# mightypirate1/DRL-Tetris

Hardware: AMD Instinct MI355X
Metric: env-steps/sec at 64k parallel 20x10 boards (higher is better)
Workload: dtype u32

## Files before the change

drl-tetris_amd/csrc/tetris_engine.h:

```cpp
#pragma once
#include "tetris_layout.h"
#include "tetris_tables.h"

#if defined(__clang__)
#define TE_UNROLL _Pragma("unroll")
#else
#define TE_UNROLL _Pragma("GCC unroll 8")
#endif

namespace te {

TE_HD int ctz32(uint32_t v) { return __builtin_ctz(v); }
TE_HD int clz32(uint32_t v) { return __builtin_clz(v); }
#if defined(__HIP_DEVICE_COMPILE__)
TE_HD uint32_t ld_stream(const uint32_t* p) { return __builtin_nontemporal_load(p); }
TE_HD void st_stream(uint32_t* p, uint32_t v) { __builtin_nontemporal_store(v, p); }
#else
TE_HD uint32_t ld_stream(const uint32_t* p) { return *p; }
TE_HD void st_stream(uint32_t* p, uint32_t v) { *p = v; }
#endif

#if defined(TE_PATH_COUNTERS) && !defined(__HIPCC__)
enum PathCounter { PC_KICK = 0, PC_KICK_2ND, PC_KICK_3RD, PC_KICK_FAILED, PC_KICK_DOWN, PC_DROP_EXACT, PC_RT_OFF_SPAWN,
                   PC_GARBAGE_ROW, PC_GARBAGE_LIFT2, PC_DEATH_GARBAGE, PC_DEATH_SPAWN, PC_TIMER_LOCK, PC_KEY_KICK, PC_KEY_KICK_FAILED,
// ... 38 lines not shown
    if (mem != MEM_STREAM) st_agent(p, v); else st_stream(p, v);
}
#endif
TE_HD uint32_t ldw(const uint32_t* base, uint32_t o, size_t word_off, int mem = MEM_STREAM) { return ldw_b(base, o, word_off * 4u, mem); }
TE_HD void stw(uint32_t* base, uint32_t o, size_t word_off, uint32_t v, int mem = MEM_STREAM) { stw_b(base, o, word_off * 4u, v, mem); }
struct RowStride { size_t ws; };
template <int N>
struct RowTable { uint32_t bytes[N]; };
TE_HD size_t row_bytes(const RowStride& r, int w) { return (size_t)w * r.ws * 4u; }
template <int N>
TE_HD size_t row_bytes(const RowTable<N>& r, int w) { return r.bytes[w]; }
#if defined(__HIP_DEVICE_COMPILE__)
TE_HD void add_word(uint32_t* p, uint32_t v) { (void)__hip_atomic_fetch_add(p, v, __ATOMIC_RELAXED, __HIP_MEMORY_SCOPE_AGENT); }
#else
TE_HD void add_word(uint32_t* p, uint32_t v) { *p += v; }
#endif
#if defined(__HIP_DEVICE_COMPILE__)
TE_HD uint32_t mul24(uint32_t a, uint32_t b) { return __umul24(a, b); }
#else
TE_HD uint32_t mul24(uint32_t a, uint32_t b) { return a * b; }
#endif
TE_HD int imin(int a, int b) { return a < b ? a : b; }
TE_HD int imax(int a, int b) { return a > b ? a : b; }
TE_HD uint32_t f2u(float f) { union { float f; uint32_t u; } v; v.f = f; return v.u; }
TE_HD float u2f(uint32_t u) { union { float f; uint32_t u; } v; v.u = u; return v.f; }

constexpr uint16_t SHAPE_ROWS[7][4] = {
    {0x2260, 0x0710, 0x3220, 0x4700}, {0x2230, 0x1700, 0x6220, 0x0740}, {0x2640, 0x0630, 0x1320, 0x6300},
    {0x2310, 0x3600, 0x4620, 0x0360}, {0x2222, 0x0f00, 0x4444, 0x00f0}, {0x0720, 0x2320, 0x2700, 0x2620},
    {0x0660, 0x0660, 0x0660, 0x0660},
};
TE_HD int spawn_rot(int kind) { return (int)((0x0977u >> (2 * (kind & 7))) & 3u); }
TE_HD int shape_value(int kind) { return (int)((0x06127534u >> (4 * (kind & 7))) & 15u); }

constexpr uint32_t make_shape(int kind, int rot) {
    uint32_t rows = SHAPE_ROWS[kind][rot];
    uint32_t nibs = 0;
    for (int gy = 0; gy < 4; gy++) {
        uint32_t rown = (rows >> (4 * (3 - gy))) & 0xF;
        for (int gx = 0; gx < 4; gx++)
            if ((rown >> gx) & 1) nibs |= 1u << (4 * gx + gy);
    }
    int minc = 3, maxc = 0;
    for (int gx = 0; gx < 4; gx++)
        if ((nibs >> (4 * gx)) & 0xF) { if (gx < minc) minc = gx; if (gx > maxc) maxc = gx; }
    return nibs | ((uint32_t)minc << 16) | ((uint32_t)maxc << 18);
}
constexpr uint32_t make_drop_word(uint32_t nibs) {
    uint32_t w = 0;
    for (int gx = 0; gx < 4; gx++) {
        uint32_t n = (nibs >> (4 * gx)) & 0xF;
        int bottom = -1;
        for (int gy = 0; gy < 4; gy++)
            if ((n >> gy) & 1) bottom = gy;
        w |= (uint32_t)(bottom < 0 ? 0x7F : 0x40 - (bottom + 1)) << (8 * gx);
    }
    return w;
}
constexpr int SHAPE_WORDS = 64;
struct ShapeTable { uint32_t s[SHAPE_WORDS]; };
constexpr ShapeTable make_shape_table() {
    ShapeTable t{};
    for (int k = 0; k < 7; k++)
        for (int r = 0; r < 4; r++) {
            t.s[k * 4 + r] = make_shape(k, r);
            t.s[32 + k * 4 + r] = make_drop_word(t.s[k * 4 + r] & 0xFFFFu);
        }
    for (int r = 0; r < 4; r++) { t.s[28 + r] = 0; t.s[60 + r] = 0x7F7F7F7Fu; }
    return t;
}
constexpr ShapeTable SHAPES = make_shape_table();

struct Ctx {
    const uint32_t* shapes;
    const uint8_t* table;
    const uint64_t* start;
    const double* combo_pow;
    uint32_t n_draws;
    uint32_t margin;
    int H;
    uint32_t floor_bits;
    bool tint;
    bool queue;
};

constexpr int ERR_FIFO = 1;
constexpr int ERR_STREAM = 2;

struct Raw8 { uint32_t lo, hi; };
struct Player {
    uint32_t col[NCOL];
    uint32_t tint[3][NCOL];
    int kind, rot, x, y, next;
    int dead, lock_armed, reward;
    int inc_count, combo_count, line_count, qlen;
    int q_overflow;
    int32_t time_ms, drop_delay, drop_time, speedup_time, lock_time;
    int32_t combo_start, combo_time, min_remaining;
    uint32_t combo_remaining;
    float incoming;
    uint32_t piece_draws, hole_draws;
    uint32_t pgroup;
    uint32_t lines_sent, lines_cleared, lines_blocked, max_combo, lines_seen, garbage_cleared;
    int32_t qcount[FIFO_CAP];
    int32_t qdelay[FIFO_CAP];
    int q_loaded;
    Raw8 pf_raw;
    int pf_ok;
};

struct ResetPrefetch { uint32_t seed16; uint64_t word; int ok; };

template <int P>
struct Game {
    Player pl[P];
    uint32_t seed16;
    int round_over, last_winner;
    uint32_t flags;
    uint32_t episode;
    uint32_t steps;
    uint32_t add_lines, add_sent;
    uint32_t status;
    uint32_t draw0, draw1;
};

template <class ROWS>
TE_HD void load_player_rows(const uint32_t* s, uint32_t o, const ROWS& rows, Player& q, bool tint, bool queue = true, int mem = MEM_STREAM) {
    for (int c = 0; c < NCOL; c++) q.col[c] = ldw_b(s, o, row_bytes(rows, W_COL0 + c), mem);
    if (tint)
        for (int k = 0; k < 3; k++)
            for (int c = 0; c < NCOL; c++) q.tint[k][c] = ldw_b(s, o, row_bytes(rows, W_TINT0 + 10 * k + c), mem);
    uint32_t w = ldw_b(s, o, row_bytes(rows, W_PIECE), mem);
    q.kind = w & 7; q.rot = (w >> 3) & 3; q.x = (int)((w >> 5) & 15) - 4; q.y = (w >> 9) & 31;
    q.next = (w >> 14) & 7; q.dead = (w >> 17) & 1; q.lock_armed = (w >> 18) & 1; q.reward = (w >> 19) & 255;
    w = ldw_b(s, o, row_bytes(rows, W_MISC), mem);
    q.inc_count = w & 255; q.combo_count = (w >> 8) & 255; q.line_count = (w >> 16) & 255;
    q.qlen = (w >> 24) & 15; q.q_overflow = (w >> 28) & 3;
    if (!queue) { q.inc_count = 0; q.qlen = 0; q.q_overflow = 0; }
    q.time_ms = (int32_t)ldw_b(s, o, row_bytes(rows, W_TIME), mem);
    w = ldw_b(s, o, row_bytes(rows, W_DROPCOMBO), mem);
    q.drop_delay = w & 0xFFFF; q.combo_remaining = w >> 16;
    q.drop_time = (int32_t)ldw_b(s, o, row_bytes(rows, W_DROP_TIME), mem);
    q.speedup_time = (int32_t)ldw_b(s, o, row_bytes(rows, W_SPEEDUP_TIME), mem);
    q.lock_time = (int32_t)ldw_b(s, o, row_bytes(rows, W_LOCK_TIME), mem);
    q.combo_start = (int32_t)ldw_b(s, o, row_bytes(rows, W_COMBO_START), mem);
    q.combo_time = (int32_t)ldw_b(s, o, row_bytes(rows, W_COMBO_TIME), mem);
    q.incoming = queue ? u2f(ldw_b(s, o, row_bytes(rows, W_INCOMING), mem)) : 0.0f;
    q.min_remaining = queue ? (int32_t)ldw_b(s, o, row_bytes(rows, W_MIN_REMAINING), mem) : 1000;
    q.piece_draws = ldw_b(s, o, row_bytes(rows, W_PIECE_DRAWS), mem);
    q.hole_draws = queue ? ldw_b(s, o, row_bytes(rows, W_HOLE_DRAWS), mem) : 0u;
    q.pgroup = ldw_b(s, o, row_bytes(rows, W_PIECE_GROUP), mem);
    w = ldw_b(s, o, row_bytes(rows, W_STATS0), mem); q.lines_sent = w & 0xFFFF; q.lines_cleared = w >> 16;
    w = ldw_b(s, o, row_bytes(rows, W_STATS1), mem); q.lines_blocked = w & 0xFFFF; q.max_combo = w >> 16;
    w = ldw_b(s, o, row_bytes(rows, W_STATS2), mem); q.lines_seen = w & 0xFFFF; q.garbage_cleared = w >> 16;
    q.q_loaded = queue && q.qlen > 0;
    q.pf_ok = 0; q.pf_raw.lo = 0; q.pf_raw.hi = 0;
    if (queue)
        for (int i = 0; i < FIFO_CAP; i++) { q.qcount[i] = 0; q.qdelay[i] = 0; }
    if (q.q_loaded) {
        for (int i = 0; i < FIFO_CAP / 2; i++) {
            uint32_t cw = ldw_b(s, o, row_bytes(rows, W_FIFO_COUNT0 + i), mem);
            q.qcount[2 * i] = (int16_t)(cw & 0xFFFF);
            q.qcount[2 * i + 1] = (int16_t)(cw >> 16);
        }
        for (int i = 0; i < FIFO_CAP; i++) q.qdelay[i] = (int32_t)ldw_b(s, o, row_bytes(rows, W_FIFO_DELAY0 + i), mem);
    }
// ... 282 lines not shown
    while (amount && q.qlen) {
        int take = imin(amount, (int)q.qcount[0]);
        if (take < 1) take = 1;
        q.qcount[0] -= take; amount -= take; blocked += take;
        if (q.qcount[0] == 0) q_pop_front(q);
    }
    q.lines_blocked = (q.lines_blocked + (uint32_t)blocked) & 0xFFFFu;
    if (q.qlen) {
        if (head_delay > q.qdelay[0]) q.qdelay[0] = head_delay;
        if (freeze) q.qdelay[0] = imin(q.qdelay[0] + 450, t + q.min_remaining + 450);
    } else
        q.min_remaining = 1000;
    return amount;
}

TE_HD bool q_release(Player& q, int32_t t) {
    if (q.qlen == 0) return false;
    if (t > q.qdelay[0]) {
        int32_t next_delay = q.qdelay[0] + 450;
        if (--q.qcount[0] == 0) q_pop_front(q);
        if (q.qlen) {
            if (next_delay > q.qdelay[0]) q.qdelay[0] = next_delay;
            q.min_remaining = q.qdelay[0] - t;
        } else
            q.min_remaining = 1000;
        return true;
    }
    q.min_remaining = imin(q.min_remaining, q.qdelay[0] - t);
    return false;
}

TE_HD int q_total(const Player& q) {
    uint32_t total = 0;
    for (int i = 0; i < FIFO_CAP; i++)
        if (i < q.qlen) total += (uint32_t)q.qcount[i];
    return (int)(total & 0xFFFFu);
}


TE_HD void combo_gain(Player& q, int32_t t, int amount) {
    if (q.combo_count == 0) { q.combo_start = t; q.combo_time = 0; }
    q.combo_count = (q.combo_count + 1) & 255;
    float line_time = 0.0f;
    for (int i = 0; i < amount; i++) {
        q.line_count = (q.line_count + 1) & 255;
        line_time = line_time + (float)(1000 / imax(1, q.line_count));
    }
    float add = (float)(800 / imax(1, q.combo_count)) + line_time;
    q.combo_time = (int32_t)((float)q.combo_time + add);
    if ((uint32_t)q.combo_count > q.max_combo) q.max_combo = (uint32_t)q.combo_count;
}

TE_HD int combo_expire(const Ctx& cx, Player& q, int32_t t) {
    int32_t left = q.combo_start + q.combo_time - t;
    q.combo_remaining = left < 0 ? 0u : ((uint32_t)left & 0xFFFFu);
    if (t > q.combo_start + q.combo_time && q.combo_count != 0) {
        float duration = 1.f + (float)t / 60000.f * 0.1f;
        double v = cx.combo_pow[q.combo_count] * (double)duration;
        int lines = (int)((uint32_t)(int64_t)v & 0xFFFFu);
        q.combo_count = 0;
        q.line_count = 0;
        return lines;
    }
    return 0;
}


TE_HD bool spawn_next(const Ctx& cx, Player& q, uint32_t seed16, uint32_t& status) {
    q.kind = q.next;
    q.rot = spawn_rot(q.kind);
    q.x = (NCOL - 4) / 2;
    q.y = 0;
    if (q.piece_draws + cx.margin >= cx.n_draws) {
        status |= ST_NEED_EXTEND;
        if (q.piece_draws >= cx.n_draws) status |= ST_STREAM_EXHAUSTED;
    }
    q.next = (int)((q.pgroup >> (4u * (q.piece_draws & 7u))) & 7u);
    q.piece_draws++;
    if ((q.piece_draws & 7u) == 0u) {
        q.pgroup = pack_group(q.pf_ok ? q.pf_raw : table_group_raw(cx, seed16, q.piece_draws, status));
        q.pf_ok = 0;
    }
    uint32_t shape = shape_of(cx, q.kind, q.rot);
    if (!fits_spawn_col(cx, q, shape, 0)) { stamp(cx, q, shape); TE_COUNT(PC_DEATH_SPAWN); return true; }
    return false;
}

TE_HD int score_clears(const Ctx& cx, Player& q, int cleared) {
    q.lines_cleared = (q.lines_cleared + (uint32_t)cleared) & 0xFFFFu;
    if (cleared == 0) { q.combo_time -= 200; return 0; }
    int amount = cx.queue ? q_block(q, cleared - 1, q.time_ms, true) : cleared - 1;
    q.lines_sent = (q.lines_sent + (uint32_t)amount) & 0xFFFFu;
    combo_gain(q, q.time_ms, cleared);
    return amount;
}

TE_HD void lock_piece(const Ctx& cx, Player& q) {
    uint32_t shape = shape_of(cx, q.kind, q.rot);
    q.y += drop_distance(cx, q, shape);
    stamp(cx, q, shape);
    q.drop_time = q.time_ms;
    q.lock_armed = 0;
}

TE_HD int settle(const Ctx& cx, Player& q, uint32_t seed16, uint32_t& status) {
    int sent = score_clears(cx, q, clear_rows(cx, q));
    if (spawn_next(cx, q, seed16, status)) return -1;
    return sent;
}

TE_HD bool soft_drop(const Ctx& cx, Player& q) {
    const uint32_t shape = shape_of(cx, q.kind, q.rot);
    if (q.x == (NCOL - 4) / 2 ? fits_spawn_col(cx, q, shape, q.y + 1) : fits_at(cx, q, shape, q.x, q.y + 1)) {
        q.y++;
        q.drop_time = q.time_ms;
        q.lock_armed = 0;
        return true;
    }
    if (!q.lock_armed) q.lock_time = q.time_ms + 400;
    q.lock_armed = 1;
    return false;
}

TE_HD bool gravity_due(Player& q, int32_t t) {
    if (t - q.speedup_time > 3000) {
        if (q.drop_delay > 200) q.drop_delay -= 10;
        else if (q.drop_delay > 100) q.drop_delay -= 5;
        else if (q.drop_delay > 50) q.drop_delay -= 2;
        else if (q.drop_delay > 10) q.drop_delay -= 1;
        q.speedup_time = t;
    }
    if (t - q.drop_time > q.drop_delay) { q.drop_time = t; return true; }
    return false;
}

TE_HD bool push_garbage(const Ctx& cx, Player& q, uint32_t seed16, uint32_t& status) {
    int hole = (int)(table_byte(cx, seed16, q.hole_draws, status) >> 4);
    q.hole_draws++;
    uint32_t bottom = 1u << (cx.H - 1);
    for (int c = 0; c < NCOL; c++) q.col[c] = (q.col[c] >> 1) | (c == hole ? 0u : bottom);
    if (cx.tint)
        for (int k = 0; k < 3; k++)
            for (int c = 0; c < NCOL; c++) q.tint[k][c] = (q.tint[k][c] >> 1) | (c == hole ? 0u : bottom);
    TE_COUNT(PC_GARBAGE_ROW);
    if (q.y > 0) q.y--;
    if (!fits_at(cx, q, shape_of(cx, q.kind, q.rot), q.x, q.y)) {
        if (q.y > 0) { q.y--; TE_COUNT(PC_GARBAGE_LIFT2); }
        else { TE_COUNT(PC_DEATH_GARBAGE); return true; }
    }
    return false;
}

TE_HD int tick(const Ctx& cx, Player& q, int ms, uint32_t seed16, uint32_t& status) {
    q.time_ms += ms;
    if (gravity_due(q, q.time_ms)) soft_drop(cx, q);
    int sent = 0;
    bool finished = false;
    if (q.lock_armed && q.time_ms > q.lock_time && !soft_drop(cx, q)) {
        TE_COUNT(PC_TIMER_LOCK);
        lock_piece(cx, q);
        sent = settle(cx, q, seed16, status);
        finished = true;
    }
    if (!finished) {
        if (cx.queue) {
            int whole = 0;
            while (q.incoming >= 1.0f) { whole++; q.incoming = q.incoming - 1.f; }
// ... 129 lines not shown
    out.r[0] = v.x; out.r[1] = v.y; out.r[2] = v.z; out.r[3] = v.w;
#else
    for (int i = 0; i < 4; i++) out.r[i] = cx.shapes[((kind & 7) << 2) | i];
#endif
    return out;
}
TE_HD Shapes4 drop_words_of_kind(const Ctx& cx, int kind) {
    Shapes4 out;
#if defined(__HIP_DEVICE_COMPILE__)
    const uint4 v = *reinterpret_cast<const uint4*>(cx.shapes + 32 + ((kind & 7) << 2));
    out.r[0] = v.x; out.r[1] = v.y; out.r[2] = v.z; out.r[3] = v.w;
#else
    for (int i = 0; i < 4; i++) out.r[i] = cx.shapes[32 + (((kind & 7) << 2) | i)];
#endif
    return out;
}
TE_HD uint32_t pick4(const Shapes4& s, int rot) {
    uint32_t lo = (rot & 1) ? s.r[1] : s.r[0];
    uint32_t hi = (rot & 1) ? s.r[3] : s.r[2];
    return (rot & 2) ? hi : lo;
}

TE_HD uint32_t free_positions32(uint64_t band, uint32_t shape) {
    const uint32_t lo = (uint32_t)band, hi = (uint32_t)(band >> 32), mid = (lo >> 16) | (hi << 16);
    const uint32_t s0 = shape & 0xFFFFu, s1 = s0 << 4, s2 = s0 << 8, s3 = s0 << 12, s4 = s0 << 16;
    uint32_t free = 0;
    free |= (s0 & lo) == 0 ? 1u << 0 : 0u;
    free |= (s1 & lo) == 0 ? 1u << 1 : 0u;
    free |= (s2 & lo) == 0 ? 1u << 2 : 0u;
    free |= (s3 & lo) == 0 ? 1u << 3 : 0u;
    free |= (s4 & lo) == 0 ? 1u << 4 : 0u;
    free |= (s1 & mid) == 0 ? 1u << 5 : 0u;
    free |= (s2 & mid) == 0 ? 1u << 6 : 0u;
    free |= (s3 & mid) == 0 ? 1u << 7 : 0u;
    free |= (s4 & mid) == 0 ? 1u << 8 : 0u;
    free |= (s1 & hi) == 0 ? 1u << 9 : 0u;
    free |= (s2 & hi) == 0 ? 1u << 10 : 0u;
    free |= (s3 & hi) == 0 ? 1u << 11 : 0u;
    free |= (s4 & hi) == 0 ? 1u << 12 : 0u;
    return free;
}
TE_HD uint32_t free_positions(uint64_t band, uint32_t shape) {
    const uint64_t pc = (uint64_t)(shape & 0xFFFFu);
    uint32_t free = 0;
    for (int xs = 0; xs <= 12; xs++) free |= (((pc << (4 * xs)) & band) == 0 ? 1u : 0u) << xs;
    return free;
}

TE_HD uint32_t band_win32(uint64_t band, int p) {
    const int off = 4 * p + 32;
    const uint32_t lo = (uint32_t)band, hi = (uint32_t)(band >> 32);
    const int k = off >> 5;
    const uint32_t a = k == 0 ? ~0u : (k == 1 ? lo : (k == 2 ? hi : ~0u));
    const uint32_t b = k == 0 ? lo : (k == 1 ? hi : ~0u);
#if defined(__HIP_DEVICE_COMPILE__)
    return __builtin_amdgcn_alignbit(b, a, (uint32_t)off & 31u);
#else
    const int sh = off & 31;
    return sh ? (a >> sh) | (b << (32 - sh)) : a;
#endif
}

struct RowsFrom { uint32_t v[NCOL]; };
TE_HD RowsFrom rows_from(const Ctx& cx, const Player& q, int y) {
    RowsFrom r;
    for (int c = 0; c < NCOL; c++) r.v[c] = (uint32_t)((int32_t)(q.col[c] | cx.floor_bits) >> y);
    return r;
}
TE_HD uint64_t band_of_rows(const RowsFrom& r) {
    uint32_t lo = 0xFFu, hi = 0xFFFF0000u;
    for (int c = 0; c < 6; c++) lo |= (r.v[c] & 0xFu) << (4 * c + 8);
    for (int c = 6; c < NCOL; c++) hi |= (r.v[c] & 0xFu) << (4 * (c - 6));
    return ((uint64_t)hi << 32) | lo;
}
TE_HD uint64_t band_one_down(uint64_t band, const RowsFrom& r) {
    uint32_t lo = (uint32_t)band, hi = (uint32_t)(band >> 32);
    lo = ((lo >> 1) & 0x77777777u) | 0xFFu;
    hi = ((hi >> 1) & 0x77777777u) | 0xFFFF0000u;
    for (int c = 0; c < 6; c++) lo |= (r.v[c] & 0x10u) << (4 * c + 7);
    hi |= (r.v[6] & 0x10u) >> 1;
    for (int c = 7; c < NCOL; c++) hi |= (r.v[c] & 0x10u) << (4 * (c - 6) - 1);
    return ((uint64_t)hi << 32) | lo;
}
TE_HD int drop_distance_rows(const Ctx& cx, const Player& q, const RowsFrom& r, uint32_t shape, uint32_t drop_word) {
    uint32_t d[NCOL];
    for (int c = 0; c < NCOL; c++) d[c] = (uint32_t)ctz32(r.v[c]);
    const uint32_t w0 = (d[0] << 16) | (d[1] << 24);
    const uint32_t w1 = d[2] | (d[3] << 8) | (d[4] << 16) | (d[5] << 24);
    const uint32_t w2 = d[6] | (d[7] << 8) | (d[8] << 16) | (d[9] << 24);
    const unsigned xs = (unsigned)(q.x + 2);
    const bool hi2 = (xs & 8u) != 0, hi1 = (xs & 4u) != 0;
    const uint32_t lo = hi2 ? (hi1 ? 0u : w2) : (hi1 ? w1 : w0);
    const uint32_t hi = hi2 ? 0u : (hi1 ? w2 : w1);
#if defined(__HIP_DEVICE_COMPILE__)
    const uint32_t under = __builtin_amdgcn_alignbyte(hi, lo, xs & 3u);
#else
    const uint32_t under = (uint32_t)((((uint64_t)hi << 32) | lo) >> (8 * (xs & 3u)));
#endif
    const uint32_t sum = under + drop_word;
    const uint32_t b0 = sum & 0xFFu, b1 = (sum >> 8) & 0xFFu, b2 = (sum >> 16) & 0xFFu, b3 = sum >> 24;
    const uint32_t m01 = b0 < b1 ? b0 : b1, m23 = b2 < b3 ? b2 : b3;
    const uint32_t m = m01 < m23 ? m01 : m23;
    if (m - 0x40u > 0x3Eu) { TE_COUNT(PC_DROP_EXACT); return drop_distance(cx, q, shape); }
    return (int)(m - 0x40u);
}

TE_HD void play_rt(const Ctx& cx, Player& q, int r, int t) {
    const Shapes4 sh = shapes_of_kind(cx, q.kind);
    const Shapes4 dw = drop_words_of_kind(cx, q.kind);
    if (q.y != 0 || q.x != (NCOL - 4) / 2) TE_COUNT(PC_RT_OFF_SPAWN);
    RowsFrom rows = rows_from(cx, q, q.y);
    uint64_t band = band_of_rows(rows);
    uint32_t win = band_win32(band, q.x);
    const bool fit1 = (((pick4(sh, q.rot + 1) & 0xFFFFu) << 8) & win) == 0;
    const bool fit2 = (((pick4(sh, q.rot + 2) & 0xFFFFu) << 8) & win) == 0;
    const bool fit3 = (((pick4(sh, q.rot + 3) & 0xFFFFu) << 8) & win) == 0;
    const bool easy = (r < 1 || fit1) && (r < 2 || fit2) && (r < 3 || fit3);
    if (easy) {
        q.rot = (q.rot + r) & 3;
    } else {
        int adv = fit1 ? (fit2 ? (fit3 ? 3 : 2) : 1) : 0;
        q.rot = (q.rot + adv) & 3;
        int left = r - adv;
        int kicks = 0;
        (void)kicks;
        while (left > 0) {
            const int nr = (q.rot + 1) & 3;
            const uint32_t s1 = pick4(sh, nr) & 0xFFFFu;
            const uint64_t b1 = band_one_down(band, rows);
            const uint32_t win1 = band_win32(b1, q.x);
            const uint32_t sA = s1, sB = s1 << 4, sC = s1 << 8, sD = s1 << 12, sE = s1 << 16;
            const bool k0 = (sC & win1) == 0, k1 = (sB & win) == 0, k2 = (sD & win) == 0;
            const bool k3 = (sB & win1) == 0, k4 = (sD & win1) == 0;
            const bool k5 = (sA & win) == 0, k6 = (sE & win) == 0;
            int dx = k6 ? 2 : 99, dy = 0;
            dx = k5 ? -2 : dx;
            if (k4) { dx = 1; dy = 1; }
            if (k3) { dx = -1; dy = 1; }
            if (k2) { dx = 1; dy = 0; }
            if (k1) { dx = -1; dy = 0; }
            if (k0) { dx = 0; dy = 1; }
            if (dx == 99) { TE_COUNT(PC_KICK_FAILED); break; }
            kicks++;
            TE_COUNT(kicks == 1 ? PC_KICK : (kicks == 2 ? PC_KICK_2ND : PC_KICK_3RD));
            if (dy) TE_COUNT(PC_KICK_DOWN);
            q.rot = nr; q.x += dx; q.y += dy;
            if (dy) {
                band = b1;
                for (int c = 0; c < NCOL; c++) rows.v[c] >>= 1;
            }
            left--;
            if (left > 0) {
                win = band_win32(band, q.x);
                const bool g1 = (((pick4(sh, q.rot + 1) & 0xFFFFu) << 8) & win) == 0;
                const bool g2 = left > 1 && (((pick4(sh, q.rot + 2) & 0xFFFFu) << 8) & win) == 0;
                const int more = g1 ? (g2 ? 2 : 1) : 0;
                q.rot = (q.rot + more) & 3;
                left -= more;
            }
        }
    }
    const uint32_t shape = pick4(sh, q.rot);
    const uint32_t free = free_positions32(band, shape);
    const int xs0 = q.x + 2;
    const uint32_t blocked_left = ~free & ((1u << xs0) - 1u);
    int xs = blocked_left ? 32 - clz32(blocked_left) : 0;
    const uint32_t blocked_right = (~free >> (xs + 1)) | (1u << 13);
    xs += imin(t, ctz32(blocked_right));
    q.x = xs - 2;
    q.y += drop_distance_rows(cx, q, rows, shape, pick4(dw, q.rot));
    stamp(cx, q, shape);
    q.drop_time = q.time_ms;
    q.lock_armed = 0;
}

constexpr int PROBE_PATH = 96;
struct Probe {
    Player q;
    int spawn;
    uint8_t path[PROBE_PATH]; int path_len;
    uint8_t best[PROBE_PATH]; int best_len, best_x, best_rot;
    uint8_t* keys; uint8_t* lens;
    int max_lists, max_keys, n_lists, overflow;
};
struct Pose { int rot, x, y; };
TE_HD Pose pose_get(const Probe& t) { Pose p = {t.q.rot, t.q.x, t.q.y}; return p; }
TE_HD void pose_set(Probe& t, Pose p) { t.q.rot = p.rot; t.q.x = p.x; t.q.y = p.y; }

TE_HD bool fits_any(const Ctx& cx, const Player& q, uint32_t shape, int x, int y) {
    if (y >= 0) return fits_at(cx, q, shape, x, y);
    int k = -y;
    if (k > 3) return (shape & 0xFFFFu) == 0;
    uint32_t low = ((1u << k) - 1u) * 0x1111u;
    if (shape & low) return false;
    return fits_at(cx, q, ((shape & 0xFFFFu) >> k) & ((0xFu >> k) * 0x1111u), x, 0);
}
TE_HD bool probe_fits(const Ctx& cx, const Probe& t) { return fits_any(cx, t.q, shape_of(cx, t.q.kind, t.q.rot), t.q.x, t.q.y); }
TE_HD bool probe_shift(const Ctx& cx, Probe& t, int dx) {
    if (fits_any(cx, t.q, shape_of(cx, t.q.kind, t.q.rot), t.q.x + dx, t.q.y)) { t.q.x += dx; return true; }
    return false;
}
TE_HD void probe_drop(const Ctx& cx, Probe& t) { t.q.y += drop_distance(cx, t.q, shape_of(cx, t.q.kind, t.q.rot)); }
TE_HD void path_push(Probe& t, int v) { if (t.path_len < PROBE_PATH) t.path[t.path_len++] = (uint8_t)v; else t.overflow = 1; }

TE_HD int convert_code(int m) {
    return m == 255 ? 3 : m == 254 ? 1 : m == 253 ? 6 : m == 252 ? 5 : m == 241 ? 8 : m == 242 ? 10 : m == 243 ? 9 : m;
}
TE_HD void emit_key(Probe& t, int& n, int code) {
    if (t.n_lists < t.max_lists && n < t.max_keys) t.keys[t.n_lists * t.max_keys + n] = (uint8_t)convert_code(code);
    else t.overflow = 1;
    n++;
}
TE_HD void emit_end(Probe& t, int n) {
    if (t.n_lists < t.max_lists) t.lens[t.n_lists] = (uint8_t)imin(n, t.max_keys);
    t.n_lists++;
}
TE_HD void emit_rotation(Probe& t, int& n, int value) { value &= 3; if (value) emit_key(t, n, 240 + value); }
TE_HD void emit_start_moves(Probe& t, int& n, int x) {
    const int mid = (NCOL - 4) / 2;
    for (int i = 0; i < x - mid; i++) emit_key(t, n, 255);
    for (int i = 0; i < mid - x; i++) emit_key(t, n, 254);
}

TE_HD int probe_move_up(const Ctx& cx, Probe& t) {
    t.q.y++;
    const bool landed = !probe_fits(cx, t);
    t.q.y--;
    int count = 0;
    do { t.q.y--; count++; } while (probe_fits(cx, t));
    count--;
    t.q.y++;
    if (count && landed) return 253;
    return count & 255;
}

TE_HD bool probe_commit(Probe& t) {
    for (int i = 0; i < t.path_len; i++) t.best[i] = t.path[i];
    t.best_len = t.path_len; t.best_x = t.q.x; t.best_rot = t.q.rot;
    return true;
// ... 276 lines not shown
```

drl-tetris_amd/csrc/tetris_kernels.h:

```cpp
#pragma once
#include "../../include/tetris_hip.h"
#include "tetris_engine.h"

namespace te {

struct KArgs {
    uint32_t* state;
    uint32_t* gstate;
    uint32_t* status;
    const uint8_t* table;
    const uint64_t* start;
    const double* combo_pow;
    uint32_t n_draws, margin;
    int H;
    int n_games;
    int n_stride;
    int n_players;
    int nw;
    int n;
    const int32_t* idx;
    const uint8_t* keys;
    const uint8_t* lens;
    int max_keys;
    const uint8_t* rot;
// ... 96 lines not shown
#endif
}
TE_HD bool chain_wait(const KArgs& a, uint32_t wave, bool marker) {
    const uint32_t seen = chain_poll(a, wave);
    if (seen == a.epoch - 1u) return true;
    if (!(seen & CHAIN_ABANDONED)) chain_give_up(a, wave, marker);
    return false;
}

TE_HD void chain_census(const KArgs& a, bool marker) {
#if defined(__HIP_DEVICE_COMPILE__)
    if (marker) (void)__hip_atomic_fetch_add(a.chain, 1u, __ATOMIC_RELAXED, __HIP_MEMORY_SCOPE_AGENT);
    for (uint32_t spin = 0; spin < a.chain_spin_limit; spin++) {
        if (ld_agent(a.chain) >= a.epoch) return;
        __builtin_amdgcn_s_sleep(8);
    }
    if (marker) st_agent(a.chain + CHAIN_STRIDE, 1u);
#else
    (void)a; (void)marker;
#endif
}

TE_HD Ctx make_ctx(const KArgs& a, const uint32_t* shapes, bool tint = false, bool queue = true) {
    Ctx cx;
    cx.shapes = shapes;
    cx.table = a.table;
    cx.start = a.start;
    cx.combo_pow = a.combo_pow;
    cx.n_draws = a.n_draws;
    cx.margin = a.margin;
    cx.H = a.H;
    cx.floor_bits = ~0u << a.H;
    cx.tint = tint;
    cx.queue = queue;
    return cx;
}

template <int P>
TE_HD void write_outputs(const KArgs& a, int i, const Game<P>& g, int done) {
    if (a.done) a.done[i] = (uint8_t)done;
    TE_UNROLL
    for (int p = 0; p < P; p++) {
        if (a.lines) a.lines[(size_t)p * a.n + i] = (uint8_t)g.pl[p].reward;
        if (a.dead) a.dead[(size_t)p * a.n + i] = (uint8_t)g.pl[p].dead;
    }
}

template <int P>
TE_HD void make_keys(const Ctx& cx, const KArgs& a, int i, Game<P>& g) {
    if (g.round_over) return;
    TE_UNROLL
    for (int p = 0; p < P; p++) {
        Player& q = g.pl[p];
        int len = a.lens[(size_t)p * a.n + i];
        if (q.dead) len = 0;
        for (int k = 0; k < len; k++) press_key(cx, q, a.keys[((size_t)k * P + p) * a.n + i]);
    }
}

template <int P>
TE_HD void make_rt(const Ctx& cx, Game<P>& g, int player, int r, int t) {
    if (g.round_over) return;
    TE_UNROLL
    for (int p = 0; p < P; p++)
        if (p == player && !g.pl[p].dead) play_rt(cx, g.pl[p], r, t);
}

TE_HD void policy_draw(const KArgs& a, uint32_t slot, unsigned long long step, uint32_t& w0, uint32_t& w1) {
    uint32_t w[4];
    philox4x32_10(a.policy_seed, a.game_offset + slot, (uint32_t)step, (uint32_t)(step >> 32), w);
    w0 = w[0]; w1 = w[1];
}

template <int P, int MODE, bool TINT = false, int MEM = MEM_STREAM>
TE_HD void game_load(const KArgs& a, int i, Game<P>& g) {
    const size_t slot = a.idx ? (size_t)a.idx[i] : (size_t)i;
    if (MODE != M_INIT && MODE != M_SPLIT_INIT)
        load_game<P>(geo_of(a), slot, g, TINT, P > 1 || MODE == M_SPLIT_RESET, MODE == M_ROLLOUT, MEM);
    if (MODE == M_ROLLOUT) policy_draw(a, (uint32_t)slot, a.first_step, g.draw0, g.draw1);
    if (MODE == M_STEP_RT || MODE == M_STEP_RT_AUTO) { g.draw0 = a.rot[i]; g.draw1 = (uint32_t)a.trans[i] | ((a.player ? (uint32_t)a.player[i] : 0u) << 8); }
}

template <int P>
TE_HD void rollout_step(const Ctx& cx, const KArgs& a, size_t slot, unsigned long long step, Game<P>& g, LaneCounters& cnt) {
    TE_UNROLL
    for (int p = 0; p < P; p++) prefetch_next(cx, g.pl[p], g.seed16, g.status);
    ResetPrefetch rpf;
    prefetch_reset(cx, episode_seed(a.game_offset + (uint32_t)slot, g.episode + 1), rpf);
    int r = (int)(g.draw0 & 3u), t = (int)(g.draw1 % 10u);
    int player = P > 1 ? (int)(step % (unsigned long long)P) : 0;
    uint32_t sent_before = 0;
    TE_UNROLL
    for (int p = 0; p < P; p++) sent_before += g.pl[p].lines_sent;
    make_rt<P>(cx, g, player, r, t);
    int done = finish_game<P>(cx, g, a.ms);
    cnt.steps++;
    g.steps++;
    uint32_t sent_after = 0;
    TE_UNROLL
    for (int p = 0; p < P; p++) {
        sent_after += g.pl[p].lines_sent;
        if (!g.pl[p].dead) { cnt.lines += (unsigned)g.pl[p].reward; g.add_lines += (unsigned)g.pl[p].reward; }
    }
    cnt.sent += (sent_after - sent_before) & 0xFFFFu;
    g.add_sent += (sent_after - sent_before) & 0xFFFFu;
    if (done) {
        cnt.episodes++;
        g.episode++;
        reset_game<P>(cx, g, episode_seed(a.game_offset + (uint32_t)slot, g.episode), &rpf);
    }
}

template <int P, int MODE, bool TINT = false, int MEM = MEM_STREAM>
TE_HD void game_run(const KArgs& a, int i, const uint32_t* shapes, Game<P>& g, LaneCounters& cnt) {
    const size_t slot = a.idx ? (size_t)a.idx[i] : (size_t)i;
    Ctx cx = make_ctx(a, shapes, TINT, P > 1 || MODE == M_SPLIT_INIT || MODE == M_SPLIT_RESET);
    if (MODE == M_INIT) init_game<P>(cx, g, (uint32_t)(a.seeds ? (uint16_t)a.seeds[i] : 0));
    if (MODE == M_SPLIT_INIT) {
        init_game<P>(cx, g, (uint32_t)(a.seeds ? (uint16_t)a.seeds[i] : 0));
        g.flags = SPLIT_ON | (a.steps ? SPLIT_SIDE : 0u);
    } else if (MODE == M_SPLIT_RESET) {
        if (P == 1) reset_split(cx, *reinterpret_cast<Game<1>*>(&g), (uint32_t)(a.seeds ? (uint16_t)a.seeds[i] : 0));
    } else if (MODE == M_RESET) {
        reset_game<P>(cx, g, (uint32_t)(a.seeds ? (uint16_t)a.seeds[i] : 0));
    } else if (MODE == M_RESET_SCHED) {
        g.episode++;
        reset_game<P>(cx, g, episode_seed(a.game_offset + (uint32_t)slot, g.episode));
    } else if (MODE == M_MAKE) {
        make_keys<P>(cx, a, i, g);
    } else if (MODE == M_FINISH) {
        TE_UNROLL
        for (int p = 0; p < P; p++) prefetch_next(cx, g.pl[p], g.seed16, g.status);
        int done = finish_game<P>(cx, g, a.ms);
        write_outputs<P>(a, i, g, done);
    } else if (MODE == M_STEP_KEYS) {
        TE_UNROLL
        for (int p = 0; p < P; p++) prefetch_next(cx, g.pl[p], g.seed16, g.status);
        make_keys<P>(cx, a, i, g);
        int done = finish_game<P>(cx, g, a.ms);
        write_outputs<P>(a, i, g, done);
    } else if (MODE == M_STEP_RT || MODE == M_STEP_RT_AUTO) {
        TE_UNROLL
        for (int p = 0; p < P; p++) prefetch_next(cx, g.pl[p], g.seed16, g.status);
        ResetPrefetch rpf;
        rpf.ok = 0; rpf.seed16 = 0; rpf.word = 0;
        if (MODE == M_STEP_RT_AUTO) prefetch_reset(cx, episode_seed(a.game_offset + (uint32_t)slot, g.episode + 1), rpf);
        make_rt<P>(cx, g, (int)(g.draw1 >> 8), (int)(g.draw0 & 3u), (int)(g.draw1 & 0xFFu));
        int done = finish_game<P>(cx, g, a.ms);
        write_outputs<P>(a, i, g, done);
        if (MODE == M_STEP_RT_AUTO && done) {
            g.episode++;
            reset_game<P>(cx, g, episode_seed(a.game_offset + (uint32_t)slot, g.episode), &rpf);
        }
    } else if (MODE == M_ROLLOUT) {
        for (int s = 0; s < a.steps; s++) {
            unsigned long long step = a.first_step + (unsigned long long)s;
            rollout_step<P>(cx, a, slot, step, g, cnt);
            if (s + 1 < a.steps) policy_draw(a, (uint32_t)slot, step + 1, g.draw0, g.draw1);
        }
    }
    store_game<P>(geo_of(a), slot, g, TINT, P > 1 || MODE == M_SPLIT_INIT || MODE == M_SPLIT_RESET,
                  MODE == M_ROLLOUT || MODE == M_INIT || MODE == M_SPLIT_INIT, MEM);
    report_status(a, g.status);
}

constexpr int UNDO_WORDS = 4;
constexpr uint32_t UNDO_RAN = 1u, UNDO_SIMPLE = 2u;
// ... 384 lines not shown
```

Baseline: 22.42 billion.

## Trim kick loop divergence and skip death stamp in single-player rollouts

```diff
diff --git a/drl-tetris_amd/csrc/tetris_engine.h b/drl-tetris_amd/csrc/tetris_engine.h
--- a/drl-tetris_amd/csrc/tetris_engine.h
+++ b/drl-tetris_amd/csrc/tetris_engine.h
@@ -144,6 +144,7 @@
     uint32_t floor_bits;
     bool tint;
     bool queue;
+    bool death_stamp = true;
 };
 
 constexpr int ERR_FIFO = 1;
@@ -592,7 +593,11 @@
         q.pf_ok = 0;
     }
     uint32_t shape = shape_of(cx, q.kind, q.rot);
-    if (!fits_spawn_col(cx, q, shape, 0)) { stamp(cx, q, shape); TE_COUNT(PC_DEATH_SPAWN); return true; }
+    if (!fits_spawn_col(cx, q, shape, 0)) {
+        if (cx.death_stamp) stamp(cx, q, shape);
+        TE_COUNT(PC_DEATH_SPAWN);
+        return true;
+    }
     return false;
 }
 
@@ -888,6 +893,16 @@
     for (int c = 7; c < NCOL; c++) hi |= (r.v[c] & 0x10u) << (4 * (c - 6) - 1);
     return ((uint64_t)hi << 32) | lo;
 }
+TE_HD uint64_t band_below_rows(const RowsFrom& r) {
+    uint32_t one = 1u;
+#if defined(__HIP_DEVICE_COMPILE__)
+    asm volatile("" : "+v"(one));
+#endif
+    uint32_t lo = 0xFFu, hi = 0xFFFF0000u;
+    for (int c = 0; c < 6; c++) lo |= ((r.v[c] >> one) & 0xFu) << (4 * c + 8);
+    for (int c = 6; c < NCOL; c++) hi |= ((r.v[c] >> one) & 0xFu) << (4 * (c - 6));
+    return ((uint64_t)hi << 32) | lo;
+}
 TE_HD int drop_distance_rows(const Ctx& cx, const Player& q, const RowsFrom& r, uint32_t shape, uint32_t drop_word) {
     uint32_t d[NCOL];
     for (int c = 0; c < NCOL; c++) d[c] = (uint32_t)ctz32(r.v[c]);
@@ -933,8 +948,8 @@
         while (left > 0) {
             const int nr = (q.rot + 1) & 3;
             const uint32_t s1 = pick4(sh, nr) & 0xFFFFu;
-            const uint64_t b1 = band_one_down(band, rows);
-            const uint32_t win1 = band_win32(b1, q.x);
+            uint32_t win1 = win >> 1;
+            if (s1 & 0x8888u) win1 = band_win32(band_below_rows(rows), q.x);
             const uint32_t sA = s1, sB = s1 << 4, sC = s1 << 8, sD = s1 << 12, sE = s1 << 16;
             const bool k0 = (sC & win1) == 0, k1 = (sB & win) == 0, k2 = (sD & win) == 0;
             const bool k3 = (sB & win1) == 0, k4 = (sD & win1) == 0;
@@ -946,21 +961,28 @@
             if (k2) { dx = 1; dy = 0; }
             if (k1) { dx = -1; dy = 0; }
             if (k0) { dx = 0; dy = 1; }
-            if (dx == 99) { TE_COUNT(PC_KICK_FAILED); break; }
-            kicks++;
-            TE_COUNT(kicks == 1 ? PC_KICK : (kicks == 2 ? PC_KICK_2ND : PC_KICK_3RD));
-            if (dy) TE_COUNT(PC_KICK_DOWN);
-            q.rot = nr; q.x += dx; q.y += dy;
+            const bool found = dx != 99;
+            if (!found) TE_COUNT(PC_KICK_FAILED);
+            else {
+                kicks++;
+                TE_COUNT(kicks == 1 ? PC_KICK : (kicks == 2 ? PC_KICK_2ND : PC_KICK_3RD));
+                if (dy) TE_COUNT(PC_KICK_DOWN);
+            }
+            q.rot = found ? nr : q.rot;
+            q.x += found ? dx : 0;
+            q.y += dy;
+            left = found ? left - 1 : 0;
             if (dy) {
-                band = b1;
+                band = band_one_down(band, rows);
                 for (int c = 0; c < NCOL; c++) rows.v[c] >>= 1;
             }
-            left--;
             if (left > 0) {
                 win = band_win32(band, q.x);
-                const bool g1 = (((pick4(sh, q.rot + 1) & 0xFFFFu) << 8) & win) == 0;
-                const bool g2 = left > 1 && (((pick4(sh, q.rot + 2) & 0xFFFFu) << 8) & win) == 0;
-                const int more = g1 ? (g2 ? 2 : 1) : 0;
+                const uint32_t hit1 = ((pick4(sh, q.rot + 1) & 0xFFFFu) << 8) & win;
+                const uint32_t hit2 = ((pick4(sh, q.rot + 2) & 0xFFFFu) << 8) & win;
+                const int g1 = hit1 == 0 ? 1 : 0;
+                const int g2 = g1 & (left > 1 ? 1 : 0) & (hit2 == 0 ? 1 : 0);
+                const int more = g1 + g2;
                 q.rot = (q.rot + more) & 3;
                 left -= more;
             }
diff --git a/drl-tetris_amd/csrc/tetris_kernels.h b/drl-tetris_amd/csrc/tetris_kernels.h
--- a/drl-tetris_amd/csrc/tetris_kernels.h
+++ b/drl-tetris_amd/csrc/tetris_kernels.h
@@ -202,7 +202,9 @@
 }
 
 template <int P>
-TE_HD void rollout_step(const Ctx& cx, const KArgs& a, size_t slot, unsigned long long step, Game<P>& g, LaneCounters& cnt) {
+TE_HD void rollout_step(const Ctx& cx_in, const KArgs& a, size_t slot, unsigned long long step, Game<P>& g, LaneCounters& cnt) {
+    Ctx cx = cx_in;
+    if (P == 1) cx.death_stamp = false;
     TE_UNROLL
     for (int p = 0; p < P; p++) prefetch_next(cx, g.pl[p], g.seed16, g.status);
     ResetPrefetch rpf;
diff --git a/profiles/wave_path_census.py b/profiles/wave_path_census.py
--- /dev/null
+++ b/profiles/wave_path_census.py
@@ -0,0 +1,55 @@
+import argparse
+import os
+import sys
+
+import numpy as np
+
+ROOT = os.path.dirname(os.path.dirname(os.path.abspath(__file__)))
+sys.path.insert(0, ROOT)
+
+from oracle import oracle as orc
+from tests import engines
+
+PATHS = ["kick", "kick_2nd", "kick_3rd", "kick_failed", "kick_down", "death_spawn", "drop_exact", "timer_lock"]
+LANES = 64
+
+
+def main():
+    ap = argparse.ArgumentParser()
+    ap.add_argument("--waves", type=int, default=48)
+    ap.add_argument("--warmup", type=int, default=64)
+    ap.add_argument("--steps", type=int, default=96)
+    ap.add_argument("--players", type=int, default=1)
+    ap.add_argument("--height", type=int, default=20)
+    args = ap.parse_args()
+    lanes = {k: 0 for k in PATHS + ["line_cleared"]}
+    waves = {k: 0 for k in PATHS + ["line_cleared"]}
+    kick_iterations = 0
+    for w in range(args.waves):
+        first = LANES * w
+        eng = engines.make("harness", LANES, args.players, args.height, seeds=orc.episode_seed(first + np.arange(LANES), 0))
+        eng.set_game_offset(first)
+        eng.rollout_random(args.warmup, 1)
+        engines.harness_path_counts()
+        lines = int(eng.rollout_totals()[2])
+        for s in range(args.steps):
+            eng.rollout_random(1, 1, first_step=args.warmup + s)
+            c = engines.harness_path_counts()
+            now = int(eng.rollout_totals()[2])
+            c["line_cleared"], lines = now - lines, now
+            for k in lanes:
+                lanes[k] += c[k]
+                waves[k] += 1 if c[k] else 0
+            kick_iterations += 3 if c["kick_3rd"] else 2 if c["kick_2nd"] else 1 if (c["kick"] or c["kick_failed"]) else 0
+        eng.close()
+    wave_steps = args.waves * args.steps
+    lane_steps = wave_steps * LANES
+    print(f"# {args.waves} waves x {LANES} games, {args.players} player(s), height {args.height}, {args.warmup} warm-up steps, {args.steps} counted steps")
+    print(f"# {'path':<14}{'lanes per lane-step':>22}{'waves with >= 1 such lane':>28}")
+    for k in lanes:
+        print(f"  {k:<14}{100.0 * lanes[k] / lane_steps:>20.2f} %{100.0 * waves[k] / wave_steps:>26.1f} %")
+    print(f"# kick-loop iterations per wave-step (lower bound: the deepest kick of the wave): {kick_iterations / wave_steps:.2f}")
+
+
+if __name__ == "__main__":
+    main()
```

New measurement: 22.75 billion, median of 6. +1.5%, better.
